# cwida/ALP

Measured on AMD Instinct MI355X. Metric: ALP fused decode (falp + patch) throughput, decoded doubles, higher is better.
Workload: dtype f64

## Files before the change

### alp_amd/csrc/alp_device.hpp

```cpp
#pragma once
#include <hip/hip_runtime.h>
#include <stddef.h>
#include <stdint.h>

#include "../../include/alpgpu.h"

namespace alpgpu {

constexpr int kVec        = 1024;
constexpr int kRowgroup   = 100;
constexpr int kWavesPerWg = 4;
constexpr int kFusedWaves = 8;

__device__ __constant__ const double kFracArr[21] = {
    1.0,
    0.1,
    0.01,
    0.001,
    0.0001,
    0.00001,
    0.000001,
    0.0000001,
    0.00000001,
    0.000000001,
// ... 23 lines not shown
    10000000000.0,
    100000000000.0,
    1000000000000.0,
    10000000000000.0,
    100000000000000.0,
    1000000000000000.0,
    10000000000000000.0,
    100000000000000000.0,
    1000000000000000000.0,
    10000000000000000000.0,
    100000000000000000000.0,
    1000000000000000000000.0,
    10000000000000000000000.0,
    100000000000000000000000.0,
};
__device__ __constant__ const int64_t kFactArr[19] = {1LL,
                                                      10LL,
                                                      100LL,
                                                      1000LL,
                                                      10000LL,
                                                      100000LL,
                                                      1000000LL,
                                                      10000000LL,
                                                      100000000LL,
                                                      1000000000LL,
                                                      10000000000LL,
                                                      100000000000LL,
                                                      1000000000000LL,
                                                      10000000000000LL,
                                                      100000000000000LL,
                                                      1000000000000000LL,
                                                      10000000000000000LL,
                                                      100000000000000000LL,
                                                      1000000000000000000LL};

constexpr double kMagic      = 6755399441055744.0;
constexpr double kUpperLimit = 9223372036854774784.0;
constexpr double kLowerLimit = -9223372036854774784.0;

__device__ __forceinline__ int lane_id() { return static_cast<int>(threadIdx.x) & 63; }
__device__ __forceinline__ int wave_in_wg() { return __builtin_amdgcn_readfirstlane(static_cast<int>(threadIdx.x) >> 6); }

__device__ __forceinline__ uint64_t ballot64(bool p) { return __builtin_amdgcn_ballot_w64(p); }
__device__ __forceinline__ uint32_t mbcnt64(uint64_t mask, uint32_t base) {
	return __builtin_amdgcn_mbcnt_hi(static_cast<uint32_t>(mask >> 32), __builtin_amdgcn_mbcnt_lo(static_cast<uint32_t>(mask), base));
}

__device__ __forceinline__ void wave_lds_sync() {
	__builtin_amdgcn_fence(__ATOMIC_RELEASE, "wavefront");
	__builtin_amdgcn_wave_barrier();
	__builtin_amdgcn_fence(__ATOMIC_ACQUIRE, "wavefront");
}

__device__ __forceinline__ uint32_t wave_scan_add_u32(uint32_t x) {
	int v = static_cast<int>(x);
	v += __builtin_amdgcn_update_dpp(0, v, 0x111, 0xf, 0xf, false);
	v += __builtin_amdgcn_update_dpp(0, v, 0x112, 0xf, 0xf, false);
	v += __builtin_amdgcn_update_dpp(0, v, 0x114, 0xf, 0xf, false);
	v += __builtin_amdgcn_update_dpp(0, v, 0x118, 0xf, 0xf, false);
	v += __builtin_amdgcn_update_dpp(0, v, 0x142, 0xa, 0xf, false);
	v += __builtin_amdgcn_update_dpp(0, v, 0x143, 0xc, 0xf, false);
	return static_cast<uint32_t>(v);
}

template <int CTRL, int ROW_MASK>
__device__ __forceinline__ double dpp_take_f64(double v) {
	const uint64_t b  = static_cast<uint64_t>(__double_as_longlong(v));
	int            lo = static_cast<int>(static_cast<uint32_t>(b)), hi = static_cast<int>(static_cast<uint32_t>(b >> 32));
	lo                = __builtin_amdgcn_update_dpp(0, lo, CTRL, ROW_MASK, 0xf, false);
	hi                = __builtin_amdgcn_update_dpp(0, hi, CTRL, ROW_MASK, 0xf, false);
	return __longlong_as_double(static_cast<long long>((static_cast<uint64_t>(static_cast<uint32_t>(hi)) << 32) | static_cast<uint32_t>(lo)));
}
__device__ __forceinline__ double wave_tree_sum_f64(double v) {
	v = v + dpp_take_f64<0x111, 0xf>(v);
	v = v + dpp_take_f64<0x112, 0xf>(v);
	v = v + dpp_take_f64<0x114, 0xf>(v);
	v = v + dpp_take_f64<0x118, 0xf>(v);
	v = v + dpp_take_f64<0x142, 0xa>(v);
	v = v + dpp_take_f64<0x143, 0xc>(v);
	const uint64_t b  = static_cast<uint64_t>(__double_as_longlong(v));
	const uint32_t lo = __builtin_amdgcn_readlane(static_cast<uint32_t>(b), 63), hi = __builtin_amdgcn_readlane(static_cast<uint32_t>(b >> 32), 63);
	return __longlong_as_double(static_cast<long long>((static_cast<uint64_t>(hi) << 32) | lo));
}

__device__ __forceinline__ uint64_t bw_mask(int bw) { return bw >= 64 ? ~0ULL : ((1ULL << bw) - 1ULL); }

__device__ __forceinline__ uint64_t uniform_u64(uint64_t x) {
	const uint32_t lo = __builtin_amdgcn_readfirstlane(static_cast<uint32_t>(x));
	const uint32_t hi = __builtin_amdgcn_readfirstlane(static_cast<uint32_t>(x >> 32));
	return (static_cast<uint64_t>(hi) << 32) | lo;
}

__device__ __forceinline__ alpgpu_rowgroup_state load_rowgroup_state(const alpgpu_rowgroup_state* __restrict__ p, int lane) {
	static_assert(sizeof(alpgpu_rowgroup_state) == 32, "eight words");
	const uint32_t mine = reinterpret_cast<const uint32_t*>(p)[lane & 7];
	uint32_t       w[8];
#pragma unroll
	for (int i = 0; i < 8; ++i) { w[i] = __builtin_amdgcn_readlane(mine, i); }
	alpgpu_rowgroup_state s;
	s.scheme = static_cast<uint8_t>(w[0]);
	s.k      = static_cast<uint8_t>(w[0] >> 8);
#pragma unroll
	for (int i = 0; i < 10; ++i) { s.combos[i] = static_cast<uint8_t>(w[(2 + i) >> 2] >> (8 * ((2 + i) & 3))); }
	s.rd_rbw       = static_cast<uint8_t>(w[3]);
	s.rd_lbw       = static_cast<uint8_t>(w[3] >> 8);
	s.rd_dict_size = static_cast<uint8_t>(w[3] >> 16);
// ... 143 lines not shown
```

### alp_amd/csrc/decode_f32_kernels.hip

```cpp
#include "alp_device_f32.hpp"
#include "decode_f32_device.hpp"
#include "decode_policy.hpp"
#include "launch.hpp"
#include "wave_minmax.hpp"
#include <cstdlib>

namespace alpgpu {

constexpr int kDecThreadsF  = 256;
constexpr int kStageBytesF  = 4480;
constexpr int kExcStageF    = 256;

struct __attribute__((aligned(16))) DecodeLdsF32 {
	static constexpr bool kPrefixInLds = false;
	uint8_t  stage[kStageBytesF];
	uint32_t mask[32];
	uint8_t  excv[4 * kExcStageF];
	uint16_t rdict[8];
};

struct ExcMaskF {
	uint32_t word;
	int      excl;
};
template <class LDS>
__device__ __forceinline__ ExcMaskF load_exception_mask_f32(const LDS& L, int lane) {
	ExcMaskF  m;
	m.word      = L.mask[lane & 31];
	const int c = lane < 32 ? __builtin_popcount(m.word) : 0;
	int       v = c;
	v += __builtin_amdgcn_update_dpp(0, v, 0x111, 0xf, 0xf, false);
	v += __builtin_amdgcn_update_dpp(0, v, 0x112, 0xf, 0xf, false);
	v += __builtin_amdgcn_update_dpp(0, v, 0x114, 0xf, 0xf, false);
	v += __builtin_amdgcn_update_dpp(0, v, 0x118, 0xf, 0xf, false);
	v += __builtin_amdgcn_update_dpp(0, v, 0x142, 0xa, 0xf, false);
	m.excl = v - c;
	return m;
}

template <int VAL_BYTES, class LDS>
__device__ __forceinline__ uint32_t fetch_exception_f32(const LDS& L, const uint8_t* __restrict__ rec, int rank, bool all_staged) {
	constexpr int kStaged = 4 * kExcStageF / VAL_BYTES;
	const int     at      = rank < kStaged ? rank : kStaged - 1;
	uint32_t      v;
	if constexpr (VAL_BYTES == 4) {
		v = reinterpret_cast<const uint32_t*>(L.excv)[at];
	} else {
		v = reinterpret_cast<const uint16_t*>(L.excv)[at];
	}
	asm volatile("" : "+v"(v));
	if (!all_staged) {
		if (rank >= kStaged) {
			if constexpr (VAL_BYTES == 4) {
				v = reinterpret_cast<const uint32_t*>(rec)[rank];
			} else {
				v = reinterpret_cast<const uint16_t*>(rec)[rank];
			}
		}
	}
	return v;
}

template <bool NT_STORE>
__device__ __forceinline__ void store_quad(float* __restrict__ p, const u32x4& bits) {
	if constexpr (NT_STORE) {
		__builtin_nontemporal_store(bits, reinterpret_cast<u32x4*>(p));
	} else {
		*reinterpret_cast<u32x4*>(p) = bits;
	}
}

__device__ __forceinline__ uint32_t issue_vector_loads_f32(DecodeLdsF32& L, const alpgpu_vector_desc& d, const uint8_t* __restrict__ packed,
                                                           const uint8_t* __restrict__ rec, int tid, int wave) {
	typedef unsigned long long ull2 __attribute__((ext_vector_type(2)));
	const bool  is_alp  = d.scheme == ALPGPU_SCHEME_ALP;
	const int   n_units = 8 * (d.bw + (is_alp ? 0 : d.lbw));
	const ull2* g       = reinterpret_cast<const ull2*>(packed + d.packed_off);
#pragma unroll
	for (int j = 0; j < 2; ++j) {
		const int c = tid + kDecThreadsF * j;
		if (c < n_units) { __builtin_amdgcn_global_load_lds(g + c, reinterpret_cast<ull2*>(L.stage) + (kDecThreadsF * j + 64 * wave), 16, 0, 0); }
	}
	uint32_t  pos = 0u;
	const int cnt = d.exc_cnt;
	if (cnt > 0) {
		const uint32_t val_bytes = (is_alp ? 4u : 2u) * static_cast<uint32_t>(cnt);
		const int      dwords    = static_cast<int>(((val_bytes < 4u * kExcStageF ? val_bytes : 4u * kExcStageF) + 3u) >> 2);
		static_assert(kExcStageF <= kDecThreadsF, "one load per thread covers the stage");
		if (tid < dwords) { __builtin_amdgcn_global_load_lds(reinterpret_cast<const uint32_t*>(rec) + tid, reinterpret_cast<uint32_t*>(L.excv) + 64 * wave, 4, 0, 0); }
		if (tid < cnt) { pos = reinterpret_cast<const uint16_t*>(rec + val_bytes)[tid]; }
	}
	return pos;
}

__device__ __forceinline__ void land_exceptions_f32(DecodeLdsF32& L, const alpgpu_vector_desc& d, const uint8_t* __restrict__ rec, uint32_t pos, int tid) {
	const int cnt = d.exc_cnt;
	if (tid < cnt) { atomicOr(&L.mask[pos >> 5], 1u << (pos & 31)); }
	if (cnt > kDecThreadsF) {
		const uint16_t* poss = reinterpret_cast<const uint16_t*>(rec + static_cast<size_t>(cnt) * (d.scheme == ALPGPU_SCHEME_ALP ? 4 : 2));
		for (int j = tid + kDecThreadsF; j < cnt; j += kDecThreadsF) {
			const uint32_t p = poss[j];
			atomicOr(&L.mask[p >> 5], 1u << (p & 31));
		}
	}
}

__device__ __forceinline__ RdDict load_vector_consts_f32(const alpgpu_rowgroup_state* __restrict__ rgs, uint64_t v, const alpgpu_vector_desc& d) {
	if (d.scheme != ALPGPU_SCHEME_ALP) { return load_rd_dict(rgs, v, true); }
	return RdDict {static_cast<uint64_t>(kFactArrF[d.f]), static_cast<uint64_t>(__float_as_uint(kFracArrF[d.e]))};
}

constexpr int kSinkStoreF = 0, kSinkSumF = 1, kSinkCountF = 2;
constexpr int kSinkMinMaxF = 3;
__device__ __constant__ const uint32_t kShortcutBoundF[11] = {16777216u, 16777216u, 16777216u, 2147483u, 214748u, 21474u, 2147u, 214u, 21u, 2u, 0u};
template <bool NT_STORE, int SINK, class LDS, bool HBM_EXC = true>
__device__ __forceinline__ void finish_quad_f32(const LDS& L, const QuadWords& w, const alpgpu_vector_desc& d, const RdDict& dict, const ExcMaskF& em,
                                                const uint8_t* __restrict__ rec, float* __restrict__ dst, int tid, int wave, int lane, double* acc,
                                                float range_lo, float range_hi, float* mm = nullptr) {
	const int bw   = d.bw;
	const int cnt  = d.exc_cnt;
	const int a    = tid & 7;
	const int row  = tid >> 3;
	uint32_t  hits = 0;
	int       rank = 0;
	const bool all_staged = !HBM_EXC || cnt <= (d.scheme == ALPGPU_SCHEME_ALP ? kExcStageF : 2 * kExcStageF);
	constexpr bool kApart = SINK != kSinkStoreF;
	if (kApart && cnt > 0 && d.scheme == ALPGPU_SCHEME_ALP) {
		const int wi = 8 * wave + (lane >> 3);
		uint32_t  word;
		if constexpr (LDS::kPrefixInLds) {
			word = L.mask[wi];
		} else {
			word = static_cast<uint32_t>(__shfl(static_cast<int>(em.word), wi));
		}
		hits = (word >> (4 * a)) & 0xFu;
	} else if (cnt > 0) {
		const int wi = 8 * wave + (lane >> 3);
		uint32_t  word;
		int       pref;
		if constexpr (LDS::kPrefixInLds) {
			word = L.mask[wi];
			pref = static_cast<int>(L.pref[wi]);
		} else {
			word = static_cast<uint32_t>(__shfl(static_cast<int>(em.word), wi));
			pref = __shfl(em.excl, wi);
		}
		const int      b0   = 4 * a;
		hits                = (word >> b0) & 0xFu;
		rank                = pref + __builtin_popcount(word & ((1u << b0) - 1u));
	}
	const uint32_t s    = static_cast<uint32_t>(row * bw) & 31u;
	const uint32_t msk  = bw_mask32(bw);
	u32x4          q;
// ... 53 lines not shown
#pragma unroll
		for (int c = 0; c < 4; ++c) { *acc += static_cast<double>(__uint_as_float(out[c])); }
	} else if constexpr (SINK == kSinkCountF) {
#pragma unroll
		for (int c = 0; c < 4; ++c) {
			const float v = __uint_as_float(out[c]);
			*acc += (v >= range_lo && v <= range_hi) ? 1.0 : 0.0;
		}
	} else if constexpr (SINK == kSinkMinMaxF) {
#pragma unroll
		for (int c = 0; c < 4; ++c) { minmax_take(mm[0], mm[1], __uint_as_float(out[c])); }
	} else {
		store_quad<NT_STORE>(dst + 4 * tid, out);
		if constexpr (HBM_EXC) {
			asm volatile("; quad stored (exception values beyond the stage possible)" ::: "memory");
		} else {
			asm volatile("; quad stored (exception values all staged)" ::: "memory");
		}
	}
}

template <int SINK, class LDS>
__device__ __forceinline__ void sink_exception_values_f32(const LDS& L, const uint8_t* __restrict__ rec, int cnt, int lane, double& total, float range_lo, float range_hi) {
	for (int j = lane; j < cnt; j += 64) {
		uint32_t bits;
		if (j < kExcStageF) {
			bits = reinterpret_cast<const uint32_t*>(L.excv)[j];
		} else {
			bits = reinterpret_cast<const uint32_t*>(rec)[j];
		}
		const float v = __uint_as_float(bits);
		if constexpr (SINK == kSinkCountF) {
			total += (v >= range_lo && v <= range_hi) ? 1.0 : 0.0;
		} else {
			total += static_cast<double>(v);
		}
	}
}

template <class LDS>
__device__ __forceinline__ void minmax_exception_values_f32(const LDS& L, const uint8_t* __restrict__ rec, int cnt, int lane, float& mn, float& mx) {
	for (int j = lane; j < cnt; j += 64) {
		uint32_t bits;
		if (j < kExcStageF) {
			bits = reinterpret_cast<const uint32_t*>(L.excv)[j];
		} else {
			bits = reinterpret_cast<const uint32_t*>(rec)[j];
		}
		minmax_take(mn, mx, __uint_as_float(bits));
	}
}

template <bool NT_STORE, int SINK = kSinkStoreF>
__device__ __forceinline__ void decode_staged_vector_f32(const DecodeLdsF32& L, const alpgpu_vector_desc& d, const RdDict& dict,
                                                         const uint8_t* __restrict__ rec, float* __restrict__ dst, int tid, int wave, int lane,
                                                         double* acc = nullptr, float range_lo = 0.0f, float range_hi = 0.0f) {
	ExcMaskF em {0u, 0};
	if (d.exc_cnt > 0) { em = load_exception_mask_f32(L, lane); }
	const QuadWords w = request_quad_f32(StagedWordsF {L.stage}, d, tid);
	if (SINK == kSinkStoreF && d.exc_cnt <= (d.scheme == ALPGPU_SCHEME_ALP ? kExcStageF : 2 * kExcStageF)) {
		finish_quad_f32<NT_STORE, SINK, DecodeLdsF32, false>(L, w, d, dict, em, rec, dst, tid, wave, lane, acc, range_lo, range_hi);
	} else {
		finish_quad_f32<NT_STORE, SINK, DecodeLdsF32, true>(L, w, d, dict, em, rec, dst, tid, wave, lane, acc, range_lo, range_hi);
	}
}

template <int V, bool NT_STORE, int SINK = kSinkStoreF>
__global__ __launch_bounds__(kDecThreadsF) void k_decode_column_f32(const alpgpu_vector_desc* __restrict__ descs,
                                                                    const alpgpu_rowgroup_state* __restrict__ rgs, const uint8_t* __restrict__ packed,
                                                                    const uint8_t* __restrict__ excs, float* __restrict__ out, uint64_t n_vectors,
                                                                    uint64_t wg_offset, float range_lo, float range_hi, uint64_t* __restrict__ progress, uint64_t progress_tag,
                                                                    uint32_t gate) {
	__shared__ DecodeLdsF32 L[V];
	const int      tid  = static_cast<int>(threadIdx.x);
	const int      lane = tid & 63;
	const int      wave = wave_in_wg();
	const uint64_t v0   = (wg_offset + blockIdx.x) * V;
	if (v0 >= n_vectors) { return; }
	if constexpr (SINK == kSinkStoreF) {
		if (gate != 0u && progress[kCtxWordShape] != static_cast<uint64_t>(gate)) { return; }
		if (progress != nullptr && (blockIdx.x & 127u) == 0 && tid == 0) { __hip_atomic_store(progress, progress_tag | v0, __ATOMIC_RELAXED, __HIP_MEMORY_SCOPE_AGENT); }
	}

	alpgpu_vector_desc d[V];
	uint32_t           pos[V];
#pragma unroll
	for (int i = 0; i < V; ++i) {
		const uint64_t v = v0 + i < n_vectors ? v0 + i : v0;
		d[i]             = descs[v];
	}
	RdDict dict[V];
#pragma unroll
	for (int i = 0; i < V; ++i) { dict[i] = load_vector_consts_f32(rgs, v0 + i < n_vectors ? v0 + i : v0, d[i]); }
#pragma unroll
	for (int i = 0; i < V; ++i) { pos[i] = issue_vector_loads_f32(L[i], d[i], packed, excs + d[i].exc_off, tid, wave); }
#pragma unroll
	for (int i = 0; i < V; ++i) {
		if (d[i].scheme != ALPGPU_SCHEME_ALP && tid < 4) { reinterpret_cast<uint32_t*>(L[i].rdict)[tid] = static_cast<uint32_t>((tid < 2 ? dict[i].lo : dict[i].hi) >> (32 * (tid & 1))); }
	}
	bool any_exc = false;
#pragma unroll
	for (int i = 0; i < V; ++i) { any_exc |= d[i].exc_cnt != 0; }
	if (any_exc) {
		if (tid < 32 * V) { L[tid >> 5].mask[tid & 31] = 0; }
		asm volatile("s_waitcnt lgkmcnt(0)\n\ts_barrier" ::: "memory");
#pragma unroll
		for (int i = 0; i < V; ++i) { land_exceptions_f32(L[i], d[i], excs + d[i].exc_off, pos[i], tid); }
	}
	asm volatile("s_waitcnt vmcnt(0)" ::: "memory");
	__syncthreads();
	if constexpr (SINK != kSinkStoreF) {
		double acc[V];
#pragma unroll
		for (int i = 0; i < V; ++i) {
			acc[i] = 0.0;
			if (v0 + i < n_vectors) {
				decode_staged_vector_f32<NT_STORE, SINK>(L[i], d[i], dict[i], excs + d[i].exc_off, nullptr, tid, wave, lane, &acc[i], range_lo,
				                                         range_hi);
			}
		}
		__syncthreads();
		static_assert(kStageBytesF >= 8 * kDecThreadsF && kDecThreadsF == 256, "the lane partials of a vector fit its stage; four wavefronts per vector");
#pragma unroll
		for (int i = 0; i < V; ++i) { reinterpret_cast<double*>(L[i].stage)[tid] = acc[i]; }
		__syncthreads();
		if (wave < V && v0 + wave < n_vectors) {
			const double* part  = reinterpret_cast<const double*>(L[wave].stage) + lane;
			double        total = (part[0] + part[64]) + (part[128] + part[192]);
#pragma unroll
			for (int i = 0; i < V; ++i) {
				if (wave == i && d[i].exc_cnt > 0 && d[i].scheme == ALPGPU_SCHEME_ALP) { sink_exception_values_f32<SINK>(L[i], excs + d[i].exc_off, d[i].exc_cnt, lane, total, range_lo, range_hi); }
			}
			total               = wave_tree_sum_f64(total);
			if (lane == 0) {
				if constexpr (SINK == kSinkCountF) {
					reinterpret_cast<uint32_t*>(out)[v0 + wave] = static_cast<uint32_t>(total);
				} else {
					reinterpret_cast<double*>(out)[v0 + wave] = total;
				}
			}
		}
		return;
	}
#pragma unroll
	for (int i = 0; i < V; ++i) {
		if (v0 + i < n_vectors) {
			decode_staged_vector_f32<NT_STORE>(L[i], d[i], dict[i], excs + d[i].exc_off, out + (v0 + i) * kVec, tid, wave, lane);
		}
	}
}

template <int V>
static void launch_v(hipStream_t stream, const alpgpu_column* col, float* d_out, bool nt, int pad_kib, uint64_t* progress, uint64_t tag, uint32_t gate) {
	const uint64_t n        = col->n_vectors;
	const uint64_t n_wg     = (n + V - 1) / V;
	const uint64_t kMaxGrid = 1ull << 30;
	const unsigned pad_lds = static_cast<unsigned>(pad_kib >= 0 ? pad_kib : 0) * 1024u;
	if (gate != 0 && progress == nullptr) { gate = 0; }
	for (uint64_t off = 0; off < n_wg; off += kMaxGrid) {
		const dim3 grid(static_cast<unsigned>(n_wg - off < kMaxGrid ? n_wg - off : kMaxGrid)), block(kDecThreadsF);
		if (nt) {
			hipLaunchKernelGGL((k_decode_column_f32<V, true>), grid, block, pad_lds, stream, col->d_vectors, col->d_rowgroups, col->d_packed, col->d_exc, d_out, n, off, 0.0f, 0.0f, progress, tag, gate);
		} else {
			hipLaunchKernelGGL((k_decode_column_f32<V, false>), grid, block, pad_lds, stream, col->d_vectors, col->d_rowgroups, col->d_packed, col->d_exc, d_out, n, off, 0.0f, 0.0f, progress, tag, gate);
		}
	}
}

static int launch_store_direct_f32(hipStream_t stream, const alpgpu_column* col, float* d_out, int pad_kib, uint64_t* progress, uint64_t progress_tag);
int launch_decode_column_f32(hipStream_t stream, const alpgpu_column* col, float* d_out, int vectors_per_wg, bool plain_stores, int pad_kib, uint64_t* progress, uint64_t progress_tag,
                             uint32_t gate) {
	if (col->n_vectors == 0) { return ALPGPU_OK; }
	if (vectors_per_wg == 8) { return launch_store_direct_f32(stream, col, d_out, pad_kib, progress, progress_tag); }
	if (vectors_per_wg == 1) {
		launch_v<1>(stream, col, d_out, !plain_stores, pad_kib, progress, progress_tag, gate);
	} else if (vectors_per_wg == 2) {
		launch_v<2>(stream, col, d_out, !plain_stores, pad_kib, progress, progress_tag, gate);
	} else {
		launch_v<4>(stream, col, d_out, !plain_stores, pad_kib, progress, progress_tag, gate);
	}
	return hipGetLastError() == hipSuccess ? ALPGPU_OK : ALPGPU_ERR_HIP;
}

template <int SINK, int V>
static int launch_sink_f32(hipStream_t stream, const alpgpu_column* col, void* d_result, float lo, float hi) {
	const uint64_t n = col->n_vectors;
	if (n == 0) { return ALPGPU_OK; }
	const uint64_t n_wg     = (n + V - 1) / V;
	const uint64_t kMaxGrid = 1ull << 30;
	for (uint64_t off = 0; off < n_wg; off += kMaxGrid) {
		const dim3 grid(static_cast<unsigned>(n_wg - off < kMaxGrid ? n_wg - off : kMaxGrid)), block(kDecThreadsF);
		hipLaunchKernelGGL((k_decode_column_f32<V, false, SINK>), grid, block, 0, stream, col->d_vectors, col->d_rowgroups, col->d_packed, col->d_exc,
		                   static_cast<float*>(d_result), n, off, lo, hi, static_cast<uint64_t*>(nullptr), 0ull, 0u);
	}
	return hipGetLastError() == hipSuccess ? ALPGPU_OK : ALPGPU_ERR_HIP;
}

constexpr int kSinkStageF32 = 3584;
constexpr int kSinkStageF32MaxExc = 1024;
struct __attribute__((aligned(16))) SinkWaveLdsF32 {
// ... 156 lines not shown
```

### alp_amd/csrc/decode_kernels.hip

```cpp
#include "alp_device.hpp"
#include "decode_policy.hpp"
#include "launch.hpp"
#include "wave_minmax.hpp"
#include <cstdlib>

namespace alpgpu {

constexpr int kDecWaves     = 4;
constexpr int kStepsPerWave = 8 / kDecWaves;
constexpr int kDecodeBatch  = 4;
constexpr int kStageBytes   = 8704;
constexpr int kExcStage     = 128;
constexpr uint32_t kExcStageBytes = 8u * kExcStage;

template <int STAGE, int EXC = kExcStage>
struct __attribute__((aligned(16))) DecodeLdsT {
	static constexpr bool kPrefixInLds = false;
	static constexpr int  kStage       = STAGE;
	static constexpr uint32_t kExcBytes = 8u * EXC;
	uint8_t  stage[STAGE];
	uint32_t mask[32];
	uint8_t  excv[kExcBytes];
	uint16_t rdict[8];
};
// ... 309 lines not shown
				for (int i = 0; i < kBatchRd; ++i) {
					const int m = kStepsPerWave * q0 + b + i;
					rw[i]       = request(rbw, 8 * m + r0);
					lw[i]       = units.left_pair(rbw, 32 * (((2 * m + (lane >> 5)) * lbw) >> 4) + (lane & 31));
				}
#pragma unroll
				for (int i = 0; i < kBatchRd; ++i) {
					const int      m   = kStepsPerWave * q0 + b + i;
					double*        acc_q = sink_acc<SINK>(acc, (b + i) / kStepsPerWave);
					U64Pair        u   = extract(rbw, mask, 8 * m + r0, rw[i]);
					if constexpr (ONLY == 2) { asm volatile("" : "+v"(u.x), "+v"(u.y)); }
					const int      s   = ((2 * m + (lane >> 5)) * lbw) & 15;
					const uint32_t w0 = lw[i].x, w1 = lw[i].y;
					const uint32_t i0  = (((w0 & 0xFFFFu) >> s) | ((w1 & 0xFFFFu) << (16 - s))) & lmsk;
					const uint32_t i1  = (((w0 >> 16) >> s) | ((w1 >> 16) << (16 - s))) & lmsk;
					uint64_t       l0  = L.rdict[i0 & 7u];
					uint64_t       l1  = L.rdict[i1 & 7u];
					if (EXC == 1 || (EXC == 2 && cnt > 0)) {
						const bool     staged = EXC == 1 ? true : all_staged;
						int            rank;
						uint32_t       hits;
						if constexpr (LDS::kPrefixInLds) { hits = exception_hits_lds(L, m, lane, rank); } else { hits = exception_hits(em, m, lane, rank); }
						if (hits & 1u) {
							l0 = fetch_exception<2>(L, rec, rank, staged);
							++rank;
						}
						if (hits & 2u) { l1 = fetch_exception<2>(L, rec, rank, staged); }
					}
					const double ox = __longlong_as_double(static_cast<long long>((l0 << rbw) | u.x));
					const double oy = __longlong_as_double(static_cast<long long>((l1 << rbw) | u.y));
					if constexpr (SINK != kSinkStore) {
						consume_pair<SINK>(ox, oy, acc_q, range_lo, range_hi);
						if constexpr (ONLY == 2 && SINK == kSinkMinMax) { asm volatile("" : "+v"(acc_q[1])); }
						if constexpr (ONLY == 2) { asm volatile("" : "+v"(*acc_q)); }
					} else {
						store_pair<NT_STORE>(dst + 64 * m + lane, ox, oy);
					}
				}
				if constexpr (ONLY == 2) { asm volatile("" ::: "memory"); }
			}
		};
		constexpr bool kPerVectorLoops = SINK == kSinkStore && N_Q == 1;
		if (kPerVectorLoops && cnt == 0) {
			rd_steps(ExcMode<0> {});
		} else if (kPerVectorLoops && all_staged) {
			rd_steps(ExcMode<1> {});
		} else {
			rd_steps(ExcMode<2> {});
		}
	}
}

template <bool NT_STORE, int SINK = kSinkStore, class LDS = DecodeLds>
__device__ __forceinline__ void decode_staged_vector(const LDS& L, const alpgpu_vector_desc& d, const VectorConsts& dict,
                                                     const uint8_t* __restrict__ rec, double2* __restrict__ dst, int wave, int lane, double* acc = nullptr,
                                                     double range_lo = 0.0, double range_hi = 0.0) {
	ExcMask em {0u, 0};
	if (d.exc_cnt > 0) { em = load_exception_mask(L, lane); }
	decode_vector_quarters<NT_STORE, SINK, 1>(L, StagedWords {L.stage}, d, dict, em, rec, dst, wave, lane, acc, range_lo, range_hi);
}

template <class LDS>
__device__ __forceinline__ bool vector_fits_stage(const alpgpu_vector_desc& d) {
	return 128 * (static_cast<int>(d.bw) + (d.scheme == ALPGPU_SCHEME_ALP ? 0 : static_cast<int>(d.lbw))) + 128 <= LDS::kStage;
}
template <class LDS>
__device__ __forceinline__ uint32_t issue_vector_loads(LDS& L, const alpgpu_vector_desc& d, const uint8_t* __restrict__ packed,
                                                       const uint8_t* __restrict__ rec, int tid, int wave) {
	typedef unsigned long long ull2 __attribute__((ext_vector_type(2)));
	constexpr int T       = 64 * kDecWaves;
	const bool    is_alp  = d.scheme == ALPGPU_SCHEME_ALP;
	const int     n_units = vector_fits_stage<LDS>(d) ? 8 * (d.bw + (is_alp ? 0 : d.lbw)) : 0;
	const ull2*   g       = reinterpret_cast<const ull2*>(packed + d.packed_off);
	constexpr int kMaxUnits = (LDS::kStage - 128) / 16 < 528 ? (LDS::kStage - 128) / 16 : 528;
#pragma unroll
	for (int j = 0; j < (kMaxUnits + T - 1) / T; ++j) {
		const int c = tid + T * j;
		if (c < n_units) {
			__builtin_amdgcn_global_load_lds(g + c, reinterpret_cast<ull2*>(L.stage) + (T * j + 64 * wave), 16, 0, 0);
		}
	}
	uint32_t  pos = 0u;
	const int cnt = d.exc_cnt;
	if (cnt > 0) {
		const uint32_t val_bytes = (is_alp ? 8u : 2u) * static_cast<uint32_t>(cnt);
		const int      dwords    = static_cast<int>(((val_bytes < LDS::kExcBytes ? val_bytes : LDS::kExcBytes) + 3u) >> 2);
		static_assert(LDS::kExcBytes / 4 <= 2 * T, "two loads per thread cover the stage");
		if (tid < dwords) { __builtin_amdgcn_global_load_lds(reinterpret_cast<const uint32_t*>(rec) + tid, reinterpret_cast<uint32_t*>(L.excv) + 64 * wave, 4, 0, 0); }
		if constexpr (LDS::kExcBytes / 4 > T) {
			if (tid + T < dwords) { __builtin_amdgcn_global_load_lds(reinterpret_cast<const uint32_t*>(rec) + T + tid, reinterpret_cast<uint32_t*>(L.excv) + T + 64 * wave, 4, 0, 0); }
		}
		if (tid < cnt) { pos = reinterpret_cast<const uint16_t*>(rec + val_bytes)[tid]; }
	}
	return pos;
}

template <class LDS>
__device__ __forceinline__ void land_exceptions(LDS& L, const alpgpu_vector_desc& d, const uint8_t* __restrict__ rec, uint32_t pos, int tid) {
	constexpr int T   = 64 * kDecWaves;
	const int     cnt = d.exc_cnt;
	if (tid < cnt) { atomicOr(&L.mask[pos >> 5], 1u << (pos & 31)); }
	if (cnt > T) {
		const uint16_t* poss = reinterpret_cast<const uint16_t*>(rec + static_cast<size_t>(cnt) * (d.scheme == ALPGPU_SCHEME_ALP ? 8 : 2));
		for (int j = tid + T; j < cnt; j += T) {
			const uint32_t p = poss[j];
			atomicOr(&L.mask[p >> 5], 1u << (p & 31));
		}
	}
}

template <int V, bool NT_STORE, int SINK = kSinkStore, class LDS = DecodeLds>
__global__ __launch_bounds__(64 * kDecWaves) void k_decode_column(const alpgpu_vector_desc* __restrict__ descs,
                                                                  const alpgpu_rowgroup_state* __restrict__ rgs,
                                                                  const uint8_t* __restrict__ packed,
                                                                  const uint8_t* __restrict__ excs, double* __restrict__ out,
                                                                  uint64_t n_vectors, uint64_t wg_offset, double lo, double hi, uint32_t gate_word,
                                                                  uint64_t* __restrict__ progress, uint64_t progress_tag) {
	static_assert(LDS::kStage == kStageBytes || SINK == kSinkStore, "the sinks pass their lane partials through a full stage");
	__shared__ LDS L[V];
	const int      tid  = static_cast<int>(threadIdx.x);
	const int      lane = tid & 63;
	const int      wave = wave_in_wg();
	const uint64_t v0   = (wg_offset + blockIdx.x) * V;
	if (v0 >= n_vectors) { return; }
	if (SINK == kSinkStore && (gate_word >> 8) != 0u) {
		if (progress[kCtxWordShape] != static_cast<uint64_t>(gate_word >> 8)) { return; }
	}
	if (SINK == kSinkStore && progress != nullptr && (blockIdx.x & 127u) == 0 && tid == 0) {
		__hip_atomic_store(progress, progress_tag | v0, __ATOMIC_RELAXED, __HIP_MEMORY_SCOPE_AGENT);
	}

	alpgpu_vector_desc d[V];
	uint32_t           pos[V];
#pragma unroll
	for (int i = 0; i < V; ++i) {
		const uint64_t v = v0 + i < n_vectors ? v0 + i : v0;
		d[i]             = descs[v];
	}
	VectorConsts dict[V];
#pragma unroll
	for (int i = 0; i < V; ++i) { dict[i] = load_vector_consts(rgs, v0 + i < n_vectors ? v0 + i : v0, d[i]); }
	bool no_mask[V];
#pragma unroll
	for (int i = 0; i < V; ++i) {
		no_mask[i] = false;
		pos[i]     = issue_vector_loads(L[i], d[i], packed, excs + d[i].exc_off, tid, wave);
	}
#pragma unroll
	for (int i = 0; i < V; ++i) {
		if (d[i].scheme != ALPGPU_SCHEME_ALP && tid < 4) { reinterpret_cast<uint32_t*>(L[i].rdict)[tid] = static_cast<uint32_t>((tid < 2 ? dict[i].lo : dict[i].hi) >> (32 * (tid & 1))); }
	}
	bool any_exc = false;
#pragma unroll
	for (int i = 0; i < V; ++i) { any_exc |= d[i].exc_cnt != 0 && !no_mask[i]; }
	if (any_exc) {
		if (tid < 32 * V) { L[tid >> 5].mask[tid & 31] = 0; }
		asm volatile("s_waitcnt lgkmcnt(0)\n\ts_barrier" ::: "memory");
#pragma unroll
		for (int i = 0; i < V; ++i) {
			if (!no_mask[i]) { land_exceptions(L[i], d[i], excs + d[i].exc_off, pos[i], tid); }
		}
	}
	asm volatile("s_waitcnt vmcnt(0)" ::: "memory");
	__syncthreads();

	if constexpr (SINK != kSinkStore) {
		double acc[V];
#pragma unroll
		for (int i = 0; i < V; ++i) {
			acc[i] = 0.0;
			if (v0 + i < n_vectors) {
				if constexpr (SINK == kSinkProbe) {
					const int       n_units = 8 * (d[i].bw + (d[i].scheme == ALPGPU_SCHEME_ALP ? 0 : d[i].lbw));
					const uint64_t* st      = reinterpret_cast<const uint64_t*>(L[i].stage);
					uint64_t        sum     = 0;
					for (int c = tid; c < n_units; c += 64 * kDecWaves) { sum += st[2 * c] + st[2 * c + 1]; }
					acc[i] = static_cast<double>(sum & 0xFFFFFu);
				} else {
					decode_staged_vector<NT_STORE, SINK>(L[i], d[i], dict[i], excs + d[i].exc_off, nullptr, wave, lane, &acc[i], lo, hi);
				}
			}
		}
		__syncthreads();
		static_assert(kStageBytes >= 8 * 64 * kDecWaves, "the lane partials of a vector fit its stage");
#pragma unroll
		for (int i = 0; i < V; ++i) { reinterpret_cast<double*>(L[i].stage)[64 * wave + lane] = acc[i]; }
		__syncthreads();
		if (wave < V && v0 + wave < n_vectors) {
			const double* part = reinterpret_cast<const double*>(L[wave].stage) + lane;
			static_assert(kDecWaves == 4, "the documented summation order is for 4 wavefronts per vector");
			double total = (part[0] + part[64]) + (part[128] + part[192]);
			total = wave_tree_sum_f64(total);
			if (lane == 0) {
				if constexpr (SINK == kSinkCount) {
					reinterpret_cast<uint32_t*>(out)[v0 + wave] = static_cast<uint32_t>(total);
				} else {
					out[v0 + wave] = total;
				}
			}
		}
		return;
	}
#pragma unroll
	for (int i = 0; i < V; ++i) {
		if (v0 + i < n_vectors) {
			const alpgpu_vector_desc dd = d[i];
			decode_staged_vector<NT_STORE, kSinkStore, LDS>(L[i], dd, dict[i], excs + d[i].exc_off, reinterpret_cast<double2*>(out + (v0 + i) * kVec), wave, lane);
		}
	}
}

constexpr int kSinkDirectOcc = 8;
constexpr int kSinkStage = 3584;
constexpr int kSinkStageMaxExc = 48;
struct __attribute__((aligned(16))) SinkWaveLds {
	static constexpr bool kPrefixInLds = true;
	uint8_t  stage[kSinkStage + 128];
	uint32_t mask[32];
	static constexpr uint32_t kExcBytes = kExcStageBytes;
	uint8_t  excv[kExcStageBytes];
	uint32_t pref[32];
	uint16_t rdict[8];
};
template <int SINK>
__global__ __launch_bounds__(64 * kDecWaves, kSinkDirectOcc) void k_sink_direct(const alpgpu_vector_desc* __restrict__ descs, const alpgpu_rowgroup_state* __restrict__ rgs,
                                                                   const uint8_t* __restrict__ packed, const uint8_t* __restrict__ excs, double* __restrict__ out,
                                                                   uint64_t n_vectors, uint64_t wg_offset, double lo, double hi) {
#ifdef ALPGPU_SINK_REGISTER_MARGIN
	asm volatile("" ::: "v64");
#endif
	__shared__ SinkWaveLds S[kDecWaves];
	const int      lane = static_cast<int>(threadIdx.x) & 63;
	const int      wave = wave_in_wg();
	const uint64_t v    = (wg_offset + blockIdx.x) * kDecWaves + wave;
	if (v >= n_vectors) { return; }
	SinkWaveLds&             L    = S[wave];
	const alpgpu_vector_desc d    = descs[v];
	const VectorConsts       dict = load_vector_consts(rgs, v, d);
	const uint8_t*           rec  = excs + d.exc_off;
	const bool               is_alp = d.scheme == ALPGPU_SCHEME_ALP;
	const int                cnt  = d.exc_cnt;
	ExcMask                  em {0u, 0};
	const bool staged = is_alp && 128u * d.bw <= static_cast<uint32_t>(kSinkStage) && cnt <= kSinkStageMaxExc;
	if (staged) {
		typedef unsigned long long ull2 __attribute__((ext_vector_type(2)));
		const ull2* g       = reinterpret_cast<const ull2*>(packed + d.packed_off);
		const int   n_units = 8 * d.bw;
		for (int j = 0; 64 * j < n_units; ++j) {
			if (64 * j + lane < n_units) { __builtin_amdgcn_global_load_lds(g + 64 * j + lane, reinterpret_cast<ull2*>(L.stage) + 64 * j, 16, 0, 0); }
		}
	}
	if (cnt > 0) {
		const uint32_t val_bytes = (is_alp ? 8u : 2u) * static_cast<uint32_t>(cnt);
		const int      dwords    = static_cast<int>(((val_bytes < kExcStageBytes ? val_bytes : kExcStageBytes) + 3u) >> 2);
		for (int q = 0; 64 * q < dwords; ++q) {
			if (64 * q + lane < dwords) { __builtin_amdgcn_global_load_lds(reinterpret_cast<const uint32_t*>(rec) + 64 * q + lane, reinterpret_cast<uint32_t*>(L.excv) + 64 * q, 4, 0, 0); }
		}
		if (lane < 32) { L.mask[lane] = 0u; }
		wave_lds_sync();
		const uint16_t* poss = reinterpret_cast<const uint16_t*>(rec + val_bytes);
// ... 147 lines not shown
```

Baseline: 4456.

## Stage exception positions into LDS via async loads and wait only on record loads

Exception positions are now brought into LDS with global_load_lds alongside the values: the whole record goes into the exception stage when it fits, or the tail spills into the unused part of the packed stage. Record loads are issued before the packed-bit loads, so a partial vmcnt wait lets the mask be built while the packed data is still in flight. The mask bits are set with ds_or_b32, and the exception mask prefix is loaded once before decode. The aim is to avoid a blocking per-thread global load of positions on the critical path, at the cost of an extra barrier and more complex routing logic.

```diff
diff --git a/alp_amd/csrc/alp_device.hpp b/alp_amd/csrc/alp_device.hpp
--- a/alp_amd/csrc/alp_device.hpp
+++ b/alp_amd/csrc/alp_device.hpp
@@ -99,6 +99,35 @@
 	__builtin_amdgcn_fence(__ATOMIC_ACQUIRE, "wavefront");
 }
 
+template <int MAX>
+__device__ __forceinline__ void wait_for_all_but(int n) {
+	static_assert(MAX <= 8, "one case per count");
+	if (n <= 0) {
+		asm volatile("s_waitcnt vmcnt(0)" ::: "memory");
+	} else if (n == 1) {
+		asm volatile("s_waitcnt vmcnt(1)" ::: "memory");
+	} else if (n == 2 || MAX == 2) {
+		asm volatile("s_waitcnt vmcnt(2)" ::: "memory");
+	} else if (n == 3 || MAX == 3) {
+		asm volatile("s_waitcnt vmcnt(3)" ::: "memory");
+	} else if (n == 4 || MAX == 4) {
+		asm volatile("s_waitcnt vmcnt(4)" ::: "memory");
+	} else if (n == 5 || MAX == 5) {
+		asm volatile("s_waitcnt vmcnt(5)" ::: "memory");
+	} else if (n == 6 || MAX == 6) {
+		asm volatile("s_waitcnt vmcnt(6)" ::: "memory");
+	} else if (n == 7 || MAX == 7) {
+		asm volatile("s_waitcnt vmcnt(7)" ::: "memory");
+	} else {
+		asm volatile("s_waitcnt vmcnt(8)" ::: "memory");
+	}
+}
+
+__device__ __forceinline__ void lds_or_b32(uint32_t* word, uint32_t bits) {
+	const uint32_t at = static_cast<uint32_t>(reinterpret_cast<uintptr_t>((__attribute__((address_space(3))) uint32_t*)word));
+	asm volatile("ds_or_b32 %0, %1" ::"v"(at), "v"(bits) : "memory");
+}
+
 __device__ __forceinline__ uint32_t wave_scan_add_u32(uint32_t x) {
 	int v = static_cast<int>(x);
 	v += __builtin_amdgcn_update_dpp(0, v, 0x111, 0xf, 0xf, false);
diff --git a/alp_amd/csrc/decode_f32_kernels.hip b/alp_amd/csrc/decode_f32_kernels.hip
--- a/alp_amd/csrc/decode_f32_kernels.hip
+++ b/alp_amd/csrc/decode_f32_kernels.hip
@@ -70,35 +70,75 @@
 	}
 }
 
-__device__ __forceinline__ uint32_t issue_vector_loads_f32(DecodeLdsF32& L, const alpgpu_vector_desc& d, const uint8_t* __restrict__ packed,
-                                                           const uint8_t* __restrict__ rec, int tid, int wave) {
+constexpr int kRecWholeF = 0, kRecTailF = 1, kRecStreamF = 2;
+struct RecordTailF {
+	int at;
+	int dwords;
+	int skip;
+};
+__device__ __forceinline__ RecordTailF record_tail_f32(const alpgpu_vector_desc& d) {
+	const int skip = d.scheme == ALPGPU_SCHEME_ALP ? 0 : (2 * static_cast<int>(d.exc_cnt)) & 3;
+	return RecordTailF {128 * (static_cast<int>(d.bw) + (d.scheme == ALPGPU_SCHEME_ALP ? 0 : static_cast<int>(d.lbw))) + 128, (skip + 2 * static_cast<int>(d.exc_cnt) + 3) >> 2, skip};
+}
+__device__ __forceinline__ int record_route_f32(const alpgpu_vector_desc& d) {
+	if ((d.scheme == ALPGPU_SCHEME_ALP ? 6u : 4u) * static_cast<uint32_t>(d.exc_cnt) <= 4u * kExcStageF) { return kRecWholeF; }
+	const RecordTailF t = record_tail_f32(d);
+	return t.at + 4 * t.dwords <= kStageBytesF ? kRecTailF : kRecStreamF;
+}
+__device__ __forceinline__ void issue_record_loads_f32(DecodeLdsF32& L, const alpgpu_vector_desc& d, const uint8_t* __restrict__ rec, int tid, int wave) {
+	const int cnt = d.exc_cnt;
+	if (cnt > 0) {
+		const uint32_t val_bytes = (d.scheme == ALPGPU_SCHEME_ALP ? 4u : 2u) * static_cast<uint32_t>(cnt);
+		const int      route     = record_route_f32(d);
+		const uint32_t bytes     = route == kRecWholeF ? val_bytes + 2u * static_cast<uint32_t>(cnt) : (val_bytes < 4u * kExcStageF ? val_bytes : 4u * kExcStageF);
+		const int      dwords    = static_cast<int>((bytes + 3u) >> 2);
+		static_assert(kExcStageF <= kDecThreadsF, "one load per thread covers the stage");
+		if (tid < dwords) { __builtin_amdgcn_global_load_lds(reinterpret_cast<const uint32_t*>(rec) + tid, reinterpret_cast<uint32_t*>(L.excv) + 64 * wave, 4, 0, 0); }
+		if (route == kRecTailF) {
+			const RecordTailF t   = record_tail_f32(d);
+			const uint32_t*   src = reinterpret_cast<const uint32_t*>(rec + (val_bytes & ~3u));
+			uint32_t*         dst = reinterpret_cast<uint32_t*>(L.stage + t.at);
+#pragma unroll
+			for (int k = 0; k < 2; ++k) {
+				if (tid + kDecThreadsF * k < t.dwords) { __builtin_amdgcn_global_load_lds(src + tid + kDecThreadsF * k, dst + kDecThreadsF * k + 64 * wave, 4, 0, 0); }
+			}
+		}
+	}
+}
+__device__ __forceinline__ void issue_packed_loads_f32(DecodeLdsF32& L, const alpgpu_vector_desc& d, const uint8_t* __restrict__ packed, int tid, int wave) {
 	typedef unsigned long long ull2 __attribute__((ext_vector_type(2)));
-	const bool  is_alp  = d.scheme == ALPGPU_SCHEME_ALP;
-	const int   n_units = 8 * (d.bw + (is_alp ? 0 : d.lbw));
+	const int   n_units = 8 * (d.bw + (d.scheme == ALPGPU_SCHEME_ALP ? 0 : d.lbw));
 	const ull2* g       = reinterpret_cast<const ull2*>(packed + d.packed_off);
 #pragma unroll
 	for (int j = 0; j < 2; ++j) {
 		const int c = tid + kDecThreadsF * j;
 		if (c < n_units) { __builtin_amdgcn_global_load_lds(g + c, reinterpret_cast<ull2*>(L.stage) + (kDecThreadsF * j + 64 * wave), 16, 0, 0); }
 	}
-	uint32_t  pos = 0u;
-	const int cnt = d.exc_cnt;
-	if (cnt > 0) {
-		const uint32_t val_bytes = (is_alp ? 4u : 2u) * static_cast<uint32_t>(cnt);
-		const int      dwords    = static_cast<int>(((val_bytes < 4u * kExcStageF ? val_bytes : 4u * kExcStageF) + 3u) >> 2);
-		static_assert(kExcStageF <= kDecThreadsF, "one load per thread covers the stage");
-		if (tid < dwords) { __builtin_amdgcn_global_load_lds(reinterpret_cast<const uint32_t*>(rec) + tid, reinterpret_cast<uint32_t*>(L.excv) + 64 * wave, 4, 0, 0); }
-		if (tid < cnt) { pos = reinterpret_cast<const uint16_t*>(rec + val_bytes)[tid]; }
-	}
-	return pos;
-}
-
-__device__ __forceinline__ void land_exceptions_f32(DecodeLdsF32& L, const alpgpu_vector_desc& d, const uint8_t* __restrict__ rec, uint32_t pos, int tid) {
-	const int cnt = d.exc_cnt;
-	if (tid < cnt) { atomicOr(&L.mask[pos >> 5], 1u << (pos & 31)); }
-	if (cnt > kDecThreadsF) {
-		const uint16_t* poss = reinterpret_cast<const uint16_t*>(rec + static_cast<size_t>(cnt) * (d.scheme == ALPGPU_SCHEME_ALP ? 4 : 2));
-		for (int j = tid + kDecThreadsF; j < cnt; j += kDecThreadsF) {
+}
+__device__ __forceinline__ int packed_loads_of_wave_f32(const alpgpu_vector_desc& d, int wave) {
+	return (8 * (d.bw + (d.scheme == ALPGPU_SCHEME_ALP ? 0 : d.lbw)) - 64 * wave + kDecThreadsF - 1) / kDecThreadsF;
+}
+
+__device__ __forceinline__ void land_exceptions_f32(DecodeLdsF32& L, const alpgpu_vector_desc& d, const uint8_t* __restrict__ rec, int tid) {
+	const int      cnt       = d.exc_cnt;
+	const uint32_t val_bytes = (d.scheme == ALPGPU_SCHEME_ALP ? 4u : 2u) * static_cast<uint32_t>(cnt);
+	const int      route     = record_route_f32(d);
+	if (route == kRecWholeF) {
+		static_assert(kExcStageF <= kDecThreadsF, "one position per thread");
+		if (tid < cnt) {
+			const uint32_t p = reinterpret_cast<const uint16_t*>(L.excv + val_bytes)[tid];
+			lds_or_b32(&L.mask[p >> 5], 1u << (p & 31));
+		}
+	} else if (route == kRecTailF) {
+		const RecordTailF t      = record_tail_f32(d);
+		const uint16_t*   staged = reinterpret_cast<const uint16_t*>(L.stage + t.at + t.skip);
+		for (int j = tid; j < cnt; j += kDecThreadsF) {
+			const uint32_t p = staged[j];
+			lds_or_b32(&L.mask[p >> 5], 1u << (p & 31));
+		}
+	} else {
+		const uint16_t* poss = reinterpret_cast<const uint16_t*>(rec + val_bytes);
+		for (int j = tid; j < cnt; j += kDecThreadsF) {
 			const uint32_t p = poss[j];
 			atomicOr(&L.mask[p >> 5], 1u << (p & 31));
 		}
@@ -258,11 +298,9 @@
 }
 
 template <bool NT_STORE, int SINK = kSinkStoreF>
-__device__ __forceinline__ void decode_staged_vector_f32(const DecodeLdsF32& L, const alpgpu_vector_desc& d, const RdDict& dict,
+__device__ __forceinline__ void decode_staged_vector_f32(const DecodeLdsF32& L, const alpgpu_vector_desc& d, const RdDict& dict, const ExcMaskF& em,
                                                          const uint8_t* __restrict__ rec, float* __restrict__ dst, int tid, int wave, int lane,
                                                          double* acc = nullptr, float range_lo = 0.0f, float range_hi = 0.0f) {
-	ExcMaskF em {0u, 0};
-	if (d.exc_cnt > 0) { em = load_exception_mask_f32(L, lane); }
 	const QuadWords w = request_quad_f32(StagedWordsF {L.stage}, d, tid);
 	if (SINK == kSinkStoreF && d.exc_cnt <= (d.scheme == ALPGPU_SCHEME_ALP ? kExcStageF : 2 * kExcStageF)) {
 		finish_quad_f32<NT_STORE, SINK, DecodeLdsF32, false>(L, w, d, dict, em, rec, dst, tid, wave, lane, acc, range_lo, range_hi);
@@ -289,7 +327,6 @@
 	}
 
 	alpgpu_vector_desc d[V];
-	uint32_t           pos[V];
 #pragma unroll
 	for (int i = 0; i < V; ++i) {
 		const uint64_t v = v0 + i < n_vectors ? v0 + i : v0;
@@ -299,7 +336,13 @@
 #pragma unroll
 	for (int i = 0; i < V; ++i) { dict[i] = load_vector_consts_f32(rgs, v0 + i < n_vectors ? v0 + i : v0, d[i]); }
 #pragma unroll
-	for (int i = 0; i < V; ++i) { pos[i] = issue_vector_loads_f32(L[i], d[i], packed, excs + d[i].exc_off, tid, wave); }
+	for (int i = 0; i < V; ++i) { issue_record_loads_f32(L[i], d[i], excs + d[i].exc_off, tid, wave); }
+	int behind_records = 0;
+#pragma unroll
+	for (int i = 0; i < V; ++i) {
+		issue_packed_loads_f32(L[i], d[i], packed, tid, wave);
+		behind_records += packed_loads_of_wave_f32(d[i], wave);
+	}
 #pragma unroll
 	for (int i = 0; i < V; ++i) {
 		if (d[i].scheme != ALPGPU_SCHEME_ALP && tid < 4) { reinterpret_cast<uint32_t*>(L[i].rdict)[tid] = static_cast<uint32_t>((tid < 2 ? dict[i].lo : dict[i].hi) >> (32 * (tid & 1))); }
@@ -307,11 +350,20 @@
 	bool any_exc = false;
 #pragma unroll
 	for (int i = 0; i < V; ++i) { any_exc |= d[i].exc_cnt != 0; }
+	ExcMaskF em[V];
+#pragma unroll
+	for (int i = 0; i < V; ++i) { em[i] = ExcMaskF {0u, 0}; }
 	if (any_exc) {
 		if (tid < 32 * V) { L[tid >> 5].mask[tid & 31] = 0; }
+		wait_for_all_but<2 * V>(behind_records);
 		asm volatile("s_waitcnt lgkmcnt(0)\n\ts_barrier" ::: "memory");
 #pragma unroll
-		for (int i = 0; i < V; ++i) { land_exceptions_f32(L[i], d[i], excs + d[i].exc_off, pos[i], tid); }
+		for (int i = 0; i < V; ++i) { land_exceptions_f32(L[i], d[i], excs + d[i].exc_off, tid); }
+		asm volatile("s_waitcnt lgkmcnt(0)\n\ts_barrier" ::: "memory");
+#pragma unroll
+		for (int i = 0; i < V; ++i) {
+			if (d[i].exc_cnt > 0) { em[i] = load_exception_mask_f32(L[i], lane); }
+		}
 	}
 	asm volatile("s_waitcnt vmcnt(0)" ::: "memory");
 	__syncthreads();
@@ -321,7 +373,7 @@
 		for (int i = 0; i < V; ++i) {
 			acc[i] = 0.0;
 			if (v0 + i < n_vectors) {
-				decode_staged_vector_f32<NT_STORE, SINK>(L[i], d[i], dict[i], excs + d[i].exc_off, nullptr, tid, wave, lane, &acc[i], range_lo,
+				decode_staged_vector_f32<NT_STORE, SINK>(L[i], d[i], dict[i], em[i], excs + d[i].exc_off, nullptr, tid, wave, lane, &acc[i], range_lo,
 				                                         range_hi);
 			}
 		}
@@ -351,7 +403,7 @@
 #pragma unroll
 	for (int i = 0; i < V; ++i) {
 		if (v0 + i < n_vectors) {
-			decode_staged_vector_f32<NT_STORE>(L[i], d[i], dict[i], excs + d[i].exc_off, out + (v0 + i) * kVec, tid, wave, lane);
+			decode_staged_vector_f32<NT_STORE>(L[i], d[i], dict[i], em[i], excs + d[i].exc_off, out + (v0 + i) * kVec, tid, wave, lane);
 		}
 	}
 }
diff --git a/alp_amd/csrc/decode_kernels.hip b/alp_amd/csrc/decode_kernels.hip
--- a/alp_amd/csrc/decode_kernels.hip
+++ b/alp_amd/csrc/decode_kernels.hip
@@ -385,11 +385,9 @@
 }
 
 template <bool NT_STORE, int SINK = kSinkStore, class LDS = DecodeLds>
-__device__ __forceinline__ void decode_staged_vector(const LDS& L, const alpgpu_vector_desc& d, const VectorConsts& dict,
+__device__ __forceinline__ void decode_staged_vector(const LDS& L, const alpgpu_vector_desc& d, const VectorConsts& dict, const ExcMask& em,
                                                      const uint8_t* __restrict__ rec, double2* __restrict__ dst, int wave, int lane, double* acc = nullptr,
                                                      double range_lo = 0.0, double range_hi = 0.0) {
-	ExcMask em {0u, 0};
-	if (d.exc_cnt > 0) { em = load_exception_mask(L, lane); }
 	decode_vector_quarters<NT_STORE, SINK, 1>(L, StagedWords {L.stage}, d, dict, em, rec, dst, wave, lane, acc, range_lo, range_hi);
 }
 
@@ -398,12 +396,57 @@
 	return 128 * (static_cast<int>(d.bw) + (d.scheme == ALPGPU_SCHEME_ALP ? 0 : static_cast<int>(d.lbw))) + 128 <= LDS::kStage;
 }
 template <class LDS>
-__device__ __forceinline__ uint32_t issue_vector_loads(LDS& L, const alpgpu_vector_desc& d, const uint8_t* __restrict__ packed,
-                                                       const uint8_t* __restrict__ rec, int tid, int wave) {
+__device__ __forceinline__ int staged_units(const alpgpu_vector_desc& d) {
+	return vector_fits_stage<LDS>(d) ? 8 * (d.bw + (d.scheme == ALPGPU_SCHEME_ALP ? 0 : d.lbw)) : 0;
+}
+constexpr int kRecWhole = 0, kRecTail = 1, kRecStream = 2;
+struct RecordTail {
+	int at;
+	int dwords;
+	int skip;
+};
+template <class LDS>
+__device__ __forceinline__ RecordTail record_tail(const alpgpu_vector_desc& d) {
+	const int units = staged_units<LDS>(d);
+	const int skip  = d.scheme == ALPGPU_SCHEME_ALP ? 0 : (2 * static_cast<int>(d.exc_cnt)) & 3;
+	return RecordTail {units != 0 ? 16 * units + 128 : 0, (skip + 2 * static_cast<int>(d.exc_cnt) + 3) >> 2, skip};
+}
+template <class LDS>
+__device__ __forceinline__ int record_route(const alpgpu_vector_desc& d) {
+	if ((d.scheme == ALPGPU_SCHEME_ALP ? 10u : 4u) * static_cast<uint32_t>(d.exc_cnt) <= LDS::kExcBytes) { return kRecWhole; }
+	const RecordTail t = record_tail<LDS>(d);
+	return t.at + 4 * t.dwords <= LDS::kStage ? kRecTail : kRecStream;
+}
+template <class LDS>
+__device__ __forceinline__ void issue_record_loads(LDS& L, const alpgpu_vector_desc& d, const uint8_t* __restrict__ rec, int tid, int wave) {
+	constexpr int T   = 64 * kDecWaves;
+	const int     cnt = d.exc_cnt;
+	if (cnt > 0) {
+		const uint32_t val_bytes = (d.scheme == ALPGPU_SCHEME_ALP ? 8u : 2u) * static_cast<uint32_t>(cnt);
+		const int      route     = record_route<LDS>(d);
+		const uint32_t bytes     = route == kRecWhole ? val_bytes + 2u * static_cast<uint32_t>(cnt) : (val_bytes < LDS::kExcBytes ? val_bytes : LDS::kExcBytes);
+		const int      dwords    = static_cast<int>((bytes + 3u) >> 2);
+		static_assert(LDS::kExcBytes / 4 <= 2 * T, "two loads per thread cover the stage");
+		if (tid < dwords) { __builtin_amdgcn_global_load_lds(reinterpret_cast<const uint32_t*>(rec) + tid, reinterpret_cast<uint32_t*>(L.excv) + 64 * wave, 4, 0, 0); }
+		if constexpr (LDS::kExcBytes / 4 > T) {
+			if (tid + T < dwords) { __builtin_amdgcn_global_load_lds(reinterpret_cast<const uint32_t*>(rec) + T + tid, reinterpret_cast<uint32_t*>(L.excv) + T + 64 * wave, 4, 0, 0); }
+		}
+		if (route == kRecTail) {
+			const RecordTail t   = record_tail<LDS>(d);
+			const uint32_t*  src = reinterpret_cast<const uint32_t*>(rec + (val_bytes & ~3u));
+			uint32_t*        dst = reinterpret_cast<uint32_t*>(L.stage + t.at);
+#pragma unroll
+			for (int k = 0; k < 2; ++k) {
+				if (tid + T * k < t.dwords) { __builtin_amdgcn_global_load_lds(src + tid + T * k, dst + T * k + 64 * wave, 4, 0, 0); }
+			}
+		}
+	}
+}
+template <class LDS>
+__device__ __forceinline__ void issue_packed_loads(LDS& L, const alpgpu_vector_desc& d, const uint8_t* __restrict__ packed, int tid, int wave) {
 	typedef unsigned long long ull2 __attribute__((ext_vector_type(2)));
 	constexpr int T       = 64 * kDecWaves;
-	const bool    is_alp  = d.scheme == ALPGPU_SCHEME_ALP;
-	const int     n_units = vector_fits_stage<LDS>(d) ? 8 * (d.bw + (is_alp ? 0 : d.lbw)) : 0;
+	const int     n_units = staged_units<LDS>(d);
 	const ull2*   g       = reinterpret_cast<const ull2*>(packed + d.packed_off);
 	constexpr int kMaxUnits = (LDS::kStage - 128) / 16 < 528 ? (LDS::kStage - 128) / 16 : 528;
 #pragma unroll
@@ -413,29 +456,37 @@
 			__builtin_amdgcn_global_load_lds(g + c, reinterpret_cast<ull2*>(L.stage) + (T * j + 64 * wave), 16, 0, 0);
 		}
 	}
-	uint32_t  pos = 0u;
-	const int cnt = d.exc_cnt;
-	if (cnt > 0) {
-		const uint32_t val_bytes = (is_alp ? 8u : 2u) * static_cast<uint32_t>(cnt);
-		const int      dwords    = static_cast<int>(((val_bytes < LDS::kExcBytes ? val_bytes : LDS::kExcBytes) + 3u) >> 2);
-		static_assert(LDS::kExcBytes / 4 <= 2 * T, "two loads per thread cover the stage");
-		if (tid < dwords) { __builtin_amdgcn_global_load_lds(reinterpret_cast<const uint32_t*>(rec) + tid, reinterpret_cast<uint32_t*>(L.excv) + 64 * wave, 4, 0, 0); }
-		if constexpr (LDS::kExcBytes / 4 > T) {
-			if (tid + T < dwords) { __builtin_amdgcn_global_load_lds(reinterpret_cast<const uint32_t*>(rec) + T + tid, reinterpret_cast<uint32_t*>(L.excv) + T + 64 * wave, 4, 0, 0); }
-		}
-		if (tid < cnt) { pos = reinterpret_cast<const uint16_t*>(rec + val_bytes)[tid]; }
-	}
-	return pos;
-}
-
-template <class LDS>
-__device__ __forceinline__ void land_exceptions(LDS& L, const alpgpu_vector_desc& d, const uint8_t* __restrict__ rec, uint32_t pos, int tid) {
-	constexpr int T   = 64 * kDecWaves;
-	const int     cnt = d.exc_cnt;
-	if (tid < cnt) { atomicOr(&L.mask[pos >> 5], 1u << (pos & 31)); }
-	if (cnt > T) {
-		const uint16_t* poss = reinterpret_cast<const uint16_t*>(rec + static_cast<size_t>(cnt) * (d.scheme == ALPGPU_SCHEME_ALP ? 8 : 2));
-		for (int j = tid + T; j < cnt; j += T) {
+}
+template <class LDS>
+__device__ __forceinline__ int packed_loads_of_wave(const alpgpu_vector_desc& d, int wave) {
+	return (staged_units<LDS>(d) - 64 * wave + 64 * kDecWaves - 1) / (64 * kDecWaves);
+}
+template <class LDS>
+__device__ __forceinline__ void land_exceptions(LDS& L, const alpgpu_vector_desc& d, const uint8_t* __restrict__ rec, int tid) {
+	constexpr int  T         = 64 * kDecWaves;
+	const int      cnt       = d.exc_cnt;
+	const uint32_t val_bytes = (d.scheme == ALPGPU_SCHEME_ALP ? 8u : 2u) * static_cast<uint32_t>(cnt);
+	const int      route     = record_route<LDS>(d);
+	if (route == kRecWhole) {
+		const uint16_t* staged = reinterpret_cast<const uint16_t*>(L.excv + val_bytes);
+		constexpr int   kPerThread = (static_cast<int>(LDS::kExcBytes) / 4 + T - 1) / T;
+#pragma unroll
+		for (int k = 0; k < kPerThread; ++k) {
+			if (tid + T * k < cnt) {
+				const uint32_t p = staged[tid + T * k];
+				lds_or_b32(&L.mask[p >> 5], 1u << (p & 31));
+			}
+		}
+	} else if (route == kRecTail) {
+		const RecordTail t      = record_tail<LDS>(d);
+		const uint16_t*  staged = reinterpret_cast<const uint16_t*>(L.stage + t.at + t.skip);
+		for (int j = tid; j < cnt; j += T) {
+			const uint32_t p = staged[j];
+			lds_or_b32(&L.mask[p >> 5], 1u << (p & 31));
+		}
+	} else {
+		const uint16_t* poss = reinterpret_cast<const uint16_t*>(rec + val_bytes);
+		for (int j = tid; j < cnt; j += T) {
 			const uint32_t p = poss[j];
 			atomicOr(&L.mask[p >> 5], 1u << (p & 31));
 		}
@@ -464,7 +515,6 @@
 	}
 
 	alpgpu_vector_desc d[V];
-	uint32_t           pos[V];
 #pragma unroll
 	for (int i = 0; i < V; ++i) {
 		const uint64_t v = v0 + i < n_vectors ? v0 + i : v0;
@@ -477,7 +527,13 @@
 #pragma unroll
 	for (int i = 0; i < V; ++i) {
 		no_mask[i] = false;
-		pos[i]     = issue_vector_loads(L[i], d[i], packed, excs + d[i].exc_off, tid, wave);
+		issue_record_loads(L[i], d[i], excs + d[i].exc_off, tid, wave);
+	}
+	int behind_records = 0;
+#pragma unroll
+	for (int i = 0; i < V; ++i) {
+		issue_packed_loads(L[i], d[i], packed, tid, wave);
+		behind_records += packed_loads_of_wave<LDS>(d[i], wave);
 	}
 #pragma unroll
 	for (int i = 0; i < V; ++i) {
@@ -486,12 +542,21 @@
 	bool any_exc = false;
 #pragma unroll
 	for (int i = 0; i < V; ++i) { any_exc |= d[i].exc_cnt != 0 && !no_mask[i]; }
+	ExcMask em[V];
+#pragma unroll
+	for (int i = 0; i < V; ++i) { em[i] = ExcMask {0u, 0}; }
 	if (any_exc) {
 		if (tid < 32 * V) { L[tid >> 5].mask[tid & 31] = 0; }
+		wait_for_all_but<3 * V>(behind_records);
 		asm volatile("s_waitcnt lgkmcnt(0)\n\ts_barrier" ::: "memory");
 #pragma unroll
 		for (int i = 0; i < V; ++i) {
-			if (!no_mask[i]) { land_exceptions(L[i], d[i], excs + d[i].exc_off, pos[i], tid); }
+			if (!no_mask[i]) { land_exceptions(L[i], d[i], excs + d[i].exc_off, tid); }
+		}
+		asm volatile("s_waitcnt lgkmcnt(0)\n\ts_barrier" ::: "memory");
+#pragma unroll
+		for (int i = 0; i < V; ++i) {
+			if (d[i].exc_cnt > 0) { em[i] = load_exception_mask(L[i], lane); }
 		}
 	}
 	asm volatile("s_waitcnt vmcnt(0)" ::: "memory");
@@ -510,7 +575,7 @@
 					for (int c = tid; c < n_units; c += 64 * kDecWaves) { sum += st[2 * c] + st[2 * c + 1]; }
 					acc[i] = static_cast<double>(sum & 0xFFFFFu);
 				} else {
-					decode_staged_vector<NT_STORE, SINK>(L[i], d[i], dict[i], excs + d[i].exc_off, nullptr, wave, lane, &acc[i], lo, hi);
+					decode_staged_vector<NT_STORE, SINK>(L[i], d[i], dict[i], em[i], excs + d[i].exc_off, nullptr, wave, lane, &acc[i], lo, hi);
 				}
 			}
 		}
@@ -538,7 +603,7 @@
 	for (int i = 0; i < V; ++i) {
 		if (v0 + i < n_vectors) {
 			const alpgpu_vector_desc dd = d[i];
-			decode_staged_vector<NT_STORE, kSinkStore, LDS>(L[i], dd, dict[i], excs + d[i].exc_off, reinterpret_cast<double2*>(out + (v0 + i) * kVec), wave, lane);
+			decode_staged_vector<NT_STORE, kSinkStore, LDS>(L[i], dd, dict[i], em[i], excs + d[i].exc_off, reinterpret_cast<double2*>(out + (v0 + i) * kVec), wave, lane);
 		}
 	}
 }
```

After: 4439. No clear change (-0.4%).
